# Gustavroot/DeflatedMLMC_Schwinger

Measured on AMD Instinct MI355X. Metric: hutchinson_probe_samples_per_sec_schwinger128, higher is better.
Workload: dtype f64

## Files before the change

deflatedmlmc_schwinger_amd/csrc/sw_engine.hip:

```cpp
#include "../../include/schwinger_hip.h"
#include "sw_kernels.hpp"
#include "sw_pack.hpp"
#include "sw_poly.hpp"

#include <dlfcn.h>

#include <algorithm>
#include <chrono>
#include <cmath>
#include <complex>
#include <cstdarg>
#include <cstdio>
#include <cstdlib>
#include <cstring>
#include <functional>
#include <map>
#include <mutex>
#include <string>
#include <type_traits>
#include <vector>

using swk::cplx;
using swk::cplxf;
using swk::PtrList;
// ... 158 lines not shown
  bool mfma_ops = true;
  bool mfma_3m = true;
  int mfma3_tiles = 0;
  int mfma_tiles = 4;
  int f32_tiles = 0;
  int f32_stages = 4, f32_dense_stages = 8;
  int f32_splitk = 1;
  bool f32_krylov = true;
  bool f32_pairs = true;
  int mfma_small_tiles = 2;
  int sync_hint[SW_MAX_HIER][SW_MAX_LEVELS] = {{0}};
  bool lazy_sync = true;
  int eo_skew = -1;
  bool eo_skew_chunk = false;
  bool gram_cycle = true;
  bool eo_product = true;
  int gj_block = 32;
  int eo_tile = 0;
  int dense_lds = 4;
  int eo_tile_dbg = 0;
  int num_cus = 256;
  bool direct_small = true;
  bool lgmres_aug = true;
  bool stencil_nt = false;
  int stencil_tile = 0;
  int stencil_spw = 0;
  bool cgs2 = false;
  bool verify = true;
  bool inner_cgs2 = false;
  bool pyth_last = true;
// ... 192 lines not shown
    field<&sw_engine::p_even>("p_even"),
    {"ell_order", get_field<&sw_engine::ell_order>, [](sw_engine* h, double v) {
       h->ell_order = v != 0.0;
       for (Hier& H : h->hier) H.even_valid = false;
     }},
    field<&sw_engine::direct_small>("direct_small"),
    field<&sw_engine::eo_direct>("eo_direct"),
    field<&sw_engine::lgmres_aug>("lgmres_aug"),
    field<&sw_engine::cgs2>("cgs2"),
    field<&sw_engine::inner_cgs2>("inner_cgs2"),
    field<&sw_engine::pyth_last>("pyth_last"),
    field<&sw_engine::verify>("verify"),
    field<&sw_engine::lazy_sync>("lazy_sync"),
    field<&sw_engine::eo_solve>("eo_solve"),
    field<&sw_engine::gram_cycle>("gram_cycle"),
    field<&sw_engine::stop_factor>("stop_factor", [](double v) { return v > 0.0 && v <= 1.0; },
                                   "stop_factor must be in (0, 1]"),
    field<&sw_engine::precond_f32>("precond_f32"),
    field<&sw_engine::f32_krylov>("f32_krylov"),
    field<&sw_engine::f32_pairs>("f32_pairs"),
    field<&sw_engine::f32_tiles>("f32_tiles",
                                 [](double v) { const int t = (int)v; return t == 0 || t == 1 || t == 2 || t == 4; },
                                 "f32_tiles must be 0, 1, 2 or 4"),
    field<&sw_engine::f32_stages>("f32_stages"),
    field<&sw_engine::f32_dense_stages>("f32_dense_stages"),
    field<&sw_engine::f32_splitk>("f32_splitk"),
    field<&sw_engine::bench_what>("bench_what", [](double v) { return !(v < 0.0 || v > 3.0); },
                                  "bench_what must be 0..3"),
    field<&sw_engine::bench_mode>("bench_mode", [](double v) { return v == 0.0 || v == 1.0 || v == 2.0; },
                                  "bench_mode must be 0, 1 or 2"),
// ... 901 lines not shown
      const bool even = lv.stencil ? (row < lv.n / 2) : (even_row_tile[row / 16] != 0);
      if (even) ev.push_back(g);
    }
    if (ev.empty()) continue;
    SWCHK(upload(h, &P.order_even, ev.data(), ev.size()));
    P.ngroups_even = (int)ev.size();
  }
  H.even_valid = true;
  return 0;
}

static inline int* sink_slot(sw_engine* h);
static bool f32_capable(const Hier& H, int level);

static int gram_cycle_update(sw_engine* h, const PtrList& pu, const PtrList& pz, int L, int n, int nbp, cplx* X,
                             KrylovWS& ws, swk::FgTail tg) {
  tg.kind = SW_TAIL_GRAM;
  tg.s = ws.sc;
  tg.j = L;
  tg.h1 = ws.gram;
  SWCHK(multigram(h, pu, L + 1, n, nbp, ws.gram, &tg));
  return multiaxpy(h, pz, L, ws.sc.ys, 1.0, X, X, n, nbp, nullptr);
}
static int gram_cycle(sw_engine* h, const KrylovSys& sys, const cplx* R, cplx* X, int L, KrylovWS& ws, int nbp,
                      swk::FgTail tg) {
  const size_t vec = (size_t)sys.n * nbp;
  PtrList pu, pz;
  pu.p[0] = R;
  for (int j = 0; j < L; ++j) {
    cplx* z = ws.Z + vec * j;
    cplx* w = ws.V + vec * j;
    SWCHK(sys.precond(pu.p[j], z));
    SWCHK(sys.apply(0, z, nullptr, w));
    pu.p[j + 1] = w;
    pz.p[j] = z;
  }
  return gram_cycle_update(h, pu, pz, L, sys.n, nbp, X, ws, tg);
}

static int kcycle_gram(sw_engine* h, Hier& H, int level, const cplx* B, cplx* X, int L, KrylovWS& ws, int nbp) {
  swk::FgTail tg{};
  tg.first_cycle = 1;
  tg.notconv = sink_slot(h);
  SWCHK(zero_vec(h, X, H.lv[level].n, nbp));
  return gram_cycle(h, full_system(h, H, level, nbp, true, false), B, X, L, ws, nbp, tg);
}

static int coarse_correction(sw_engine* h, Hier& H, int l, int nbp) {
  Level& lv = H.lv[l];
  Level& lc = H.lv[l + 1];
  const int last = H.nlevels - 1;
  if (lv.kcycle > 0 && l + 1 < last) {
// ... 2199 lines not shown
    return 0;
  }
  if (lv.n <= 0) return sw_fail(h, "level %d undefined", level);
  if (shift >= lv.n) return sw_fail(h, "shift %lld >= n", (long long)shift);
  std::vector<int> src(lv.n);
  for (int i = 0; i < lv.n; ++i) {
    const int s = (int)(((int64_t)i - shift + lv.n) % lv.n);
    const int ri = lv.h_rowmap.empty() ? i : lv.h_rowmap[i];
    const int rs = lv.h_rowmap.empty() ? s : lv.h_rowmap[s];
    src[ri] = rs;
  }
  SWCHK(upload(h, &h->perm_src[level], src.data(), src.size()));
  return 0;
}

int sw_set_rhsmap(sw_engine* h, int level, int n, const int64_t* indptr, const int32_t* indices,
                  const double* data) {
  SWCHK(check_hier(h, 0, level, false));
  HIPCHK(hipSetDevice(h->device));
  Level& lv = h->hier[0].lv[level];
  if (lv.n != n) return sw_fail(h, "rhs map size %d != level size %d", n, lv.n);
  SWCHK(free_op(h, h->rhsmap[level]));
  std::vector<int> rows_int;
  if (!lv.h_rowmap.empty()) {
    rows_int.resize(n);
    for (int i = 0; i < n; ++i) rows_int[lv.h_rowmap[i]] = i;
  }
  return build_ell(h, h->rhsmap[level], n, n, indptr, indices, (const std::complex<double>*)data,
                   rows_int, lv.h_rowmap, 1);
}
// ... 464 lines not shown
  if (h->precond_f32 && h->f32_krylov && f32_capable(H, 0)) {
    s.precond32 = [h, &H, nbp](const cplxf* v, cplxf* z) { return vcycle32_even(h, H, v, z, nbp); };
    s.op32 = [h, &lv, nbp](const cplxf* z, cplxf* w) { return schur_apply32(h, lv, z, w, nbp); };
  }
  return s;
}

static int reduced_rhs(sw_engine* h, Level& lv, const cplx* B, KrylovWS& ws, int nbp) {
  PtrList pl;
  pl.p[0] = B;
  const swk::FgTail tbeg = tail_begin(ws, 1);
  SWCHK(multidot(h, pl, 1, B, lv.n, nbp, ws.nrm, nullptr, nullptr, &tbeg));
  return eo_hop<0>(h, lv, B, B, ws.xacc, nbp);
}

static int fgmres_eo(sw_engine* h, Hier& H, const cplx* B, cplx* X, double tol, int maxiter, int m,
                     KrylovWS& ws, int nbp, int* iters_total) {
  Level& lv = H.lv[0];
  SWCHK(ensure_level_ws(h, lv, nbp));
  SWCHK(reduced_rhs(h, lv, B, ws, nbp));
  SWCHK(fgmres_loop(h, H, 0, reduced_system(h, H, nbp), ws.xacc, X, tol, maxiter, m, true, ws, nbp,
                    iters_total));
  return eo_hop<1>(h, lv, B, X, X, nbp);
}

static int fgmres_eo_gram(sw_engine* h, Hier& H, const cplx* B, cplx* X, double tol, int maxiter, int m,
                          KrylovWS& ws, int nbp, int* iters_total) {
  Level& lv = H.lv[0];
  const int hid_idx = (int)(&H - &h->hier[0]);
  const int hint = h->lazy_sync ? h->sync_hint[hid_idx][0] : 0;
  const KrylovSys sys = reduced_system(h, H, nbp);
  const double tol_stop = tol * h->stop_factor;
  SWCHK(ensure_level_ws(h, lv, nbp));
  SWCHK(reset_slots(h));
  SWCHK(reduced_rhs(h, lv, B, ws, nbp));
  const cplx* bp = ws.xacc;
  SWCHK(zero_vec(h, X, sys.n, nbp));
  std::vector<std::complex<double>> hrr(nbp), hrr0(nbp);
  int done = 0;
  bool converged = false;
  const cplx* Rcur = bp;
  int L = std::min(m, maxiter);
  while (done < maxiter && !converged) {
    L = std::max(1, std::min(L, std::min(m, maxiter - done)));
    int* slot = nullptr;
    SWCHK(take_slot(h, &slot));
    swk::FgTail tg{};
    tg.tol = tol;
    tg.tol_stop = tol_stop;
    tg.iter_base = done;
    tg.notconv = slot;
    SWCHK(gram_cycle(h, sys, Rcur, X, L, ws, nbp, tg));
    done += L;
    SWCHK(sys.apply(1, X, bp, ws.rres));
    Rcur = ws.rres;
    const bool observe = tol_stop > 0.0 && (hint <= 0 || done + m >= hint || done >= maxiter);
    int Lnext = m;
    if (observe) {
      int left = 0;
      SWCHK(read_slot(h, slot, &left));
      if (left == 0) {
        converged = true;
      } else {
        HIPCHK(hipMemcpy(hrr.data(), ws.sc.relres, sizeof(cplx) * nbp, hipMemcpyDeviceToHost));
        HIPCHK(hipMemcpy(hrr0.data(), ws.sc.g, sizeof(cplx) * nbp, hipMemcpyDeviceToHost));
        double need = 1.0;
        for (int c = 0; c < nbp; ++c) {
// ... 9 lines not shown
      PtrList pr;
      pr.p[0] = ws.rres;
      int* vslot = nullptr;
      SWCHK(take_slot(h, &vslot));
      const swk::FgTail tv = tail_verify(ws, tol, tol_stop, vslot);
      SWCHK(multidot(h, pr, 1, ws.rres, sys.n, nbp, ws.nrm, nullptr, nullptr, &tv));
      int left = 0;
      SWCHK(read_slot(h, vslot, &left));
      if (left != 0) {
        converged = false;
        Lnext = 1;
      }
    }
    L = Lnext;
  }
  SWCHK(eo_hop<1>(h, lv, B, X, X, nbp));
  if (iters_total) *iters_total = done;
  h->sync_hint[hid_idx][0] = converged ? done : 0;
  return 0;
}

static bool level_is_direct(sw_engine* h, Hier& H, int level) {
  return h->direct_small && level < H.nlevels - 1 && !H.lv[level].stencil && H.lv[level].dinv.set &&
         h->use_mfma;
}

static int solve_dev(sw_engine* h, int hid, int level0, const cplx* B, cplx* X, double tol,
                     int maxiter, int nbp, int* total) {
  Hier& H = h->hier[hid];
  Level& lv = H.lv[level0];
  if (level0 == H.nlevels - 1 && H.nlevels > 1) {
// ... 1726 lines not shown
  }
  return 0;
}

static int batch_tail(sw_engine* h, const Batch& b, int total, int G, std::initializer_list<ResultBuf*> results,
                      std::vector<int32_t> sum = {}) {
  SWCHK(stream_sync(h));
  for (ResultBuf* r : results) r->done(b.nb);
  sum.resize(b.nb, 0);
  SWCHK(fold_iters(h, b, total, G, sum));
  h->last_iters_f = sum;
  h->last_iters_c.assign(b.nb, 0);
  return 0;
}

static int body_hutchinson(sw_engine* h, const Batch& b) {
  int total = 0;
  SWCHK(pack_probes(h, b));
  SWCHK(fine_solve(h, b, true, &total));
  SWCHK(dot_into(h, h->pb_x0, h->pb_z, h->hier[0].lv[0].n, b.nbp, h->pb_est));
  return batch_tail(h, b, total, 1, {});
}

static int body_shifts(sw_engine* h, const Batch& b) {
  int total = 0;
  SWCHK(pack_probes(h, b));
  SWCHK(fine_solve(h, b, false, &total));
  SWCHK(shift_dots(h, h->hier[0].lv[0], h->pb_probes, b.nb, h->pb_z, b.nbp));
  HIPCHK(hipMemcpyAsync(h->pb_est, h->r_shifts.p, sizeof(cplx) * b.nbp, hipMemcpyDeviceToDevice, h->stream));
  return batch_tail(h, b, total, 1, {&h->r_shifts});
}

// ... 193 lines not shown
  if (m == std::end(kModes)) return sw_fail(h, "unknown mode %d", mode);
  if (m->level0 && level != 0) return sw_fail(h, "%s mode runs at level 0", m->level0);
  if (m->ready) SWCHK(m->ready(h, level));
  Batch b{mode, level, 0, level, h->pb_nb, h->pb_nbp, tol, maxiter};
  SWCHK(solve_hier(h, level, &b.hid));
  if (m->diff == 2 && level != 0) return sw_fail(h, "level skipping is defined for level 0 only");
  if (m->diff) SWCHK(diff_levels(h, level, m->diff == 2, &b.hid, &b.lcoarse));
  HIPCHK(hipSetDevice(h->device));
  SWCHK(ensure_probe_ws(h, b.nbp));
  SWCHK(ensure_small(h, b.nbp));
  if (h->pb_slot >= 0 && h->pb_slot < (int)h->slots.size() && h->slots[h->pb_slot].pending) {
    HIPCHK(hipStreamWaitEvent(h->stream, h->slots[h->pb_slot].ready, 0));
    h->slots[h->pb_slot].pending = false;
  }
  return m->body(h, b);
}


namespace {
struct RcclUid {
  char internal[128];
};
struct Rccl {
  void* lib = nullptr;
  int (*get_uid)(RcclUid*) = nullptr;
  int (*init_rank)(void**, int, RcclUid, int) = nullptr;
  int (*all_reduce)(const void*, void*, size_t, int, int, void*, hipStream_t) = nullptr;
  int (*destroy)(void*) = nullptr;
  bool tried = false, ok = false;
};
// ... 215 lines not shown
```

deflatedmlmc_schwinger_amd/csrc/sw_kernels.hpp:

```cpp
#pragma once
#include <hip/hip_runtime.h>
#include <stdint.h>

namespace swk {

typedef double2 cplx;

#define SW_WAVE 64
#define SW_BLOCK 256
#define SW_WAVES_PER_BLOCK 4
#define SW_SHIFT_SMALL_L 256
#define SW_SHIFT_MID_L 768
#define SW_SHIFT_MAX_L 1024

__device__ __forceinline__ cplx cmake(double a, double b) { cplx r; r.x = a; r.y = b; return r; }
__device__ __forceinline__ cplx cadd(cplx a, cplx b) { return cmake(a.x + b.x, a.y + b.y); }
__device__ __forceinline__ cplx csub(cplx a, cplx b) { return cmake(a.x - b.x, a.y - b.y); }
__device__ __forceinline__ cplx cmul(cplx a, cplx b) {
  return cmake(fma(a.x, b.x, -a.y * b.y), fma(a.x, b.y, a.y * b.x));
}
__device__ __forceinline__ cplx cmulc(cplx a, cplx b) {
  return cmake(fma(a.x, b.x, a.y * b.y), fma(a.x, b.y, -a.y * b.x));
}
__device__ __forceinline__ void cfma(cplx& acc, cplx a, cplx b) {
// ... 2114 lines not shown
  cplx s = cadd(cadd(s0, s1), cadd(s2, s3));
  if (wave > 0) red[wave - 1][lane] = s;
  __syncthreads();
  if (wave == 0) {
    s = cadd(s, red[0][lane]);
    s = cadd(s, red[1][lane]);
    s = cadd(s, red[2][lane]);
    out[(size_t)k * nbp + col] = s;
    if (svec) {
      const double q = svec[(size_t)k * nbp + col].x;
      coef[(size_t)k * nbp + col] = cmake(q * q * s.x, q * q * s.y);
    }
  }
}

template <int KT, bool NORM, class CV = cplx, class CW = cplx>
__global__ __launch_bounds__(SW_BLOCK) void k_multiaxpy(PtrListT<CV> V, int K,
                                                        const cplx* __restrict__ coef, double sign,
                                                        const CW* __restrict__ Win,
                                                        CW* __restrict__ Wout, int n, int nbp,
                                                        int rows_per_block,
                                                        cplx* __restrict__ partial,
                                                        cplxf* __restrict__ W32, RedArgs ra, FgTail tail) {
  __shared__ double redn[3][64];
  __shared__ cplx redt[NORM ? 256 : 1];
  const int wave = threadIdx.x >> 6, lane = threadIdx.x & 63;
  const size_t col = (size_t)blockIdx.y * 64 + lane;
  const int r0 = blockIdx.x * rows_per_block;
  const int r1 = min(n, r0 + rows_per_block);
  cplx c[KT];
#pragma unroll
  for (int k = 0; k < KT; ++k) {
    c[k] = cmake(0.0, 0.0);
    if (k < K) {
      const cplx t = coef[(size_t)k * nbp + col];
      c[k] = cmake(sign * t.x, sign * t.y);
    }
  }
  double nrm = 0.0;
  constexpr int UNR = (sizeof(CV) == sizeof(cplxf) && sizeof(CW) == sizeof(cplxf)) ? 4 : 2;
#pragma unroll UNR
  for (int r = r0 + wave; r < r1; r += SW_WAVES_PER_BLOCK) {
    const size_t off = (size_t)r * nbp + col;
    cplx w = widen(Win[off]);
#pragma unroll
    for (int k = 0; k < KT; ++k)
      if (k < K) cfma(w, c[k], widen(V.p[k][off]));
    Wout[off] = narrow<CW>(w);
    if (W32) W32[off] = cmake((float)w.x, (float)w.y);
    if (NORM) nrm = fma(w.x, w.x, fma(w.y, w.y, nrm));
  }
  if (NORM) {
    if (wave > 0) redn[wave - 1][lane] = nrm;
    __syncthreads();
    if (wave == 0) {
      nrm += redn[0][lane];
      nrm += redn[1][lane];
      nrm += redn[2][lane];
      st_partial(&partial[(size_t)blockIdx.x * nbp + col], cmake(nrm, 0.0), ra.tick1 != nullptr);
// ... 99 lines not shown
                                                         const cplx* __restrict__ X,
                                                         cplx* __restrict__ out, int n, int nbp) {
  const int wave = threadIdx.x >> 6, lane = threadIdx.x & 63;
  const size_t col = (size_t)blockIdx.y * 64 + lane;
  const int r = __builtin_amdgcn_readfirstlane(blockIdx.x * SW_WAVES_PER_BLOCK + wave);
  if (r >= n) return;
  const int s = srcrow ? srcrow[r] : r;
  cplx x = X[(size_t)s * nbp + col];
  const cplx* u = U + (size_t)s * ldu;
#pragma unroll 4
  for (int k = 0; k < kd; ++k) {
    const cplx ck = c[(size_t)k * nbp + col];
    cfma(x, cmake(-u[k].x, -u[k].y), ck);
  }
  out[(size_t)r * nbp + col] = x;
}

template <int KT>
__global__ __launch_bounds__(SW_BLOCK) void k_defl_gemm_dots(const cplx* __restrict__ U, int ldu,
                                                             const cplx* __restrict__ X, int n, int nbp,
                                                             int rows_per_block,
                                                             cplx* __restrict__ partial) {
  const int lane = threadIdx.x & 63, wave = threadIdx.x >> 6;
  const int k = lane >> 4, c = lane & 15;
  const int t0 = wave * KT;
  const int nt = min(KT, ldu / 16 - t0);
  if (nt <= 0) return;
  const int r0 = blockIdx.x * rows_per_block;
  const int r1 = min(n, r0 + rows_per_block);
  const size_t j = (size_t)blockIdx.y * 16 + c;
// ... 1744 lines not shown
```

deflatedmlmc_schwinger_amd/engine.py:

```python
import ctypes as C
import os
import sys

import numpy as np
import scipy.sparse as sp

_HERE = os.path.dirname(os.path.abspath(__file__))
LIB_PATH = os.path.join(_HERE, "libschwinger_hip.so")

MODE_HUTCHINSON = 0
MODE_MLMC = 1
MODE_MLMC_SKIP = 2
MODE_LEVEL = 3
MODE_HUTCHINSON_SHIFTS = 4
MODE_HUTCHINSON_LOOPS = 5
MODE_TWO_POINT = 6
MODE_MLMC_LOOPS = 7
MODE_MLMC_LOOPS_SKIP = 8
MODE_MLMC_DEFL_LOOPS = 9
MODE_MLMC_DEFL_LOOPS_SKIP = 10
MODE_TWO_POINT_LMA = 11
MODE_HUTCHINSON_LINK_LOOPS = 12
MODE_THREE_POINT = 13
MODE_TWO_POINT_SMEARED = 14
# ... 124 lines not shown
    sig("sw_setup_eo_operators", i32, vp, i32, i32, i32)
    sig("sw_apply_eo_operator", i32, vp, i32, i32, i32, i32, vp, vp)
    sig("sw_get_level_bsr", i32, vp, i32, i32, P(i32), vp, vp)
    sig("sw_setup_testvectors", i32, vp, i32, i32, i32, C.c_uint64, i32, dbl, i32, i32, vp)
    sig("sw_setup_transfer", i32, vp, i32, i32, i32, i32, vp, i32, i32, vp, vp, vp)
    sig("sw_setup_galerkin", i32, vp, i32, i32, i32, vp)
    sig("sw_get_level_dense", i32, vp, i32, i32, vp)
    sig("sw_setup_invert_coarsest", i32, vp, i32)
    sig("sw_setup_direct_level", i32, vp, i32, i32)
    sig("sw_setup_level_inverse", i32, vp, i32, i32)
    sig("sw_setup_arnoldi", i32, vp, i32, i32, i32, i32, C.c_uint64, vp)
    sig("sw_hier_end", i32, vp, i32)
    sig("sw_set_deflation", i32, vp, i32, vp)
    sig("sw_set_level_deflation", i32, vp, i32, i32, vp)
    sig("sw_set_perm", i32, vp, i32, i64)
    sig("sw_set_rhsmap", i32, vp, i32, i32, vp, vp, vp)
    sig("sw_set_solver", i32, vp, i32, i32)
    sig("sw_set_option", i32, vp, C.c_char_p, dbl)
    sig("sw_get_option", i32, vp, C.c_char_p, P(dbl))
    sig("sw_pool_trim", i32)
    sig("sw_get_coarsest_inv", i32, vp, i32, vp)
    sig("sw_eig_begin", i32, vp, i32, i32, C.c_uint64)
    sig("sw_eig_begin_wide", i32, vp, i32, i32, C.c_uint64, i32)
    sig("sw_eig_load", i32, vp, i32, i32, vp)
    sig("sw_eig_solve", i32, vp, i32, i32, i32, dbl, i32, P(i32))
    sig("sw_eig_apply_diff", i32, vp, i32, i32, i32, i32, dbl, i32, P(i32))
    sig("sw_eig_gram", i32, vp, i32, i32, vp)
    sig("sw_eig_rotate", i32, vp, i32, vp, i32, i32)
    sig("sw_eig_fetch", i32, vp, i32, i32, vp)
    sig("sw_eig_end", i32, vp)
# ... 10 lines not shown
        P(i32), vp)
    sig("sw_krylov_multiaxpy", i32, vp, i32, i32, i32, i32, i32, i32, vp, vp, dbl, vp, vp, vp, vp)
    sig("sw_krylov_scalars", i32, vp, i32, i32, i32, i32, i32, dbl, dbl, i32, vp, vp, vp, vp, vp, P(i32))
    sig("sw_solve", i32, vp, i32, i32, i32, vp, vp, dbl, i32, vp, vp)
    sig("sw_hutch_batch", i32, vp, i32, i32, i32, vp, dbl, i32, vp, vp)
    sig("sw_probes_upload", i32, vp, i32, i32, vp)
    sig("sw_probes_upload_slot", i32, vp, i32, i32, i32, vp)
    sig("sw_probes_select", i32, vp, i32)
    sig("sw_kernel_stats", i32, vp, i32, P(dbl), P(i64))
    sig("sw_kernel_work", i32, vp, i32, P(dbl))
    sig("sw_comm_unique_id", i32, vp)
    sig("sw_comm_init", i32, vp, i32, i32, vp)
    sig("sw_allreduce_stats", i32, vp, vp)
    sig("sw_comm_destroy", i32, vp)
    sig("sw_hutch_run", i32, vp, i32, i32, dbl, i32)
    sig("sw_sync", i32, vp)
    sig("sw_hutch_fetch", i32, vp, vp, vp)
    sig("sw_bench_dirac", i32, vp, i32, i32, i32, i32, P(dbl))
    sig("sw_set_profiling", i32, vp, i32)
    sig("sw_timers", i32, vp, P(dbl))
    sig("sw_timers_reset", i32, vp)
    sig("sw_launch_count", i32, vp, P(i64))
    sig("sw_mt_create", vp, C.c_uint32)
    sig("sw_mt_destroy", None, vp)
    sig("sw_mt_skip", None, vp, C.c_uint64)
    sig("sw_mt_raw", None, vp, C.c_uint64, vp)
    sig("sw_mt_rademacher", None, vp, C.c_uint64, vp)
    sig("sw_mt_z4", None, vp, C.c_uint64, vp)
    sig("sw_mt_from_state", vp, vp, i32)
    sig("sw_mt_get_state", None, vp, vp, P(i32))
# ... 39 lines not shown
    sig("sw_set_distillation_momenta", i32, vp, i32, vp)
    sig("sw_apply_laph_elementals", i32, vp, vp)
    sig("sw_distilled_two_point", i32, vp, i32, vp, dbl, i32, vp, vp, vp, vp)
    sig("sw_apply_laph_contract", i32, vp, i32, vp, vp, vp, vp)
    sig("sw_generalized_perambulators", i32, vp, i32, i32, i32, vp, i32, vp, dbl, i32, vp, vp, vp)
    sig("sw_apply_laph_generalized", i32, vp, i32, vp, i32, vp, i32, vp, i32, vp, vp)
    _lib = lib
    return lib


EXPORTED_SYMBOLS = (
    "sw_create", "sw_destroy", "sw_last_error", "sw_device_count", "sw_version", "sw_hier_begin",
    "sw_set_lattice", "sw_set_csr", "sw_set_transfer", "sw_set_coarsest_inv", "sw_set_cycle",
    "sw_set_smoother", "sw_set_gmres_smoother", "sw_set_eo_smoother", "sw_set_eo_operator", "sw_setup_eo_operators", "sw_apply_eo_operator",
    "sw_get_level_bsr", "sw_setup_testvectors", "sw_setup_transfer",
    "sw_setup_galerkin", "sw_get_level_dense", "sw_setup_invert_coarsest", "sw_setup_direct_level", "sw_setup_level_inverse", "sw_setup_arnoldi", "sw_hier_end", "sw_set_deflation", "sw_set_level_deflation", "sw_set_perm", "sw_set_rhsmap", "sw_set_solver", "sw_set_option", "sw_get_option",
    "sw_pool_trim", "sw_get_coarsest_inv", "sw_eig_begin", "sw_eig_begin_wide", "sw_eig_load", "sw_eig_solve", "sw_eig_apply_diff", "sw_eig_gram", "sw_eig_rotate", "sw_eig_fetch", "sw_eig_end",
    "sw_apply_dirac", "sw_restrict", "sw_prolong", "sw_coarsest", "sw_apply_deflation", "sw_vcycle", "sw_apply_op32", "sw_apply_op64", "sw_solve",
    "sw_krylov_multidot", "sw_krylov_gram_cycle", "sw_krylov_multiaxpy", "sw_krylov_scalars",
    "sw_hutch_batch", "sw_probes_upload", "sw_probes_upload_slot", "sw_probes_select",
    "sw_kernel_stats", "sw_kernel_work", "sw_hutch_run", "sw_sync", "sw_hutch_fetch",
    "sw_comm_unique_id", "sw_comm_init", "sw_allreduce_stats", "sw_comm_destroy",
    "sw_bench_dirac", "sw_set_profiling", "sw_timers", "sw_timers_reset", "sw_launch_count",
    "sw_mt_create", "sw_mt_destroy", "sw_mt_skip", "sw_mt_raw", "sw_mt_rademacher",
    "sw_mt_z4", "sw_mt_from_state", "sw_mt_get_state", "sw_mt_window", "sw_mt_jump",
    "sw_mt_jump_poly", "sw_mt_window_jump",
    "sw_probes_stream_set", "sw_probes_generate", "sw_probes_fetch",
    "sw_set_shifts", "sw_hutch_fetch_shifts", "sw_apply_shift_dots",
    "sw_set_loop_momenta", "sw_hutch_fetch_loops", "sw_apply_slice_dots",
    "sw_set_two_point", "sw_hutch_fetch_two_point", "sw_apply_slice_sources", "sw_apply_pair_dots",
    "sw_apply_slice_cdots", "sw_coarsest_loops", "sw_hutch_fetch_mlmc_loops", "sw_level_deflation_loops",
    "sw_meson_fields", "sw_low_mode_two_point", "sw_set_low_mode_inverse", "sw_apply_low_mode", "sw_hutch_fetch_two_point_lma",
    "sw_hutch_fetch_link_loops", "sw_apply_slice_link_dots",
    "sw_set_three_point", "sw_hutch_fetch_three_point", "sw_apply_seq_sources", "sw_apply_seq_dots",
    "sw_set_smearing", "sw_apply_smearing", "sw_hutch_fetch_two_point_smeared",
    "sw_set_distillation", "sw_perambulators", "sw_apply_laph_sources", "sw_apply_laph_project",
# ... 238 lines not shown
        Y = np.empty_like(X2)
        self._chk(self._lib.sw_apply_low_mode(self._h, X2.shape[0], _ptr(X2), _ptr(Y)), "sw_apply_low_mode")
        return Y[0] if single else Y

    def set_level_deflation(self, level, V):
        if V is None:
            self._chk(self._lib.sw_set_level_deflation(self._h, level, 0, None),
                      "sw_set_level_deflation")
            return
        V = _c128(np.asarray(V))
        self._chk(self._lib.sw_set_level_deflation(self._h, level, V.shape[1], _ptr(V)),
                  "sw_set_level_deflation")

    def set_perm(self, level, shift):
        self._chk(self._lib.sw_set_perm(self._h, level, int(shift)), "sw_set_perm")

    def set_shifts(self, shifts):
        s = np.ascontiguousarray([] if shifts is None else shifts, dtype=np.int64).ravel()
        self._chk(self._lib.sw_set_shifts(self._h, s.size, _ptr(s) if s.size else None), "sw_set_shifts")
        self._nshifts = int(s.size)

    def set_loop_momenta(self, momenta):
        p = np.ascontiguousarray([] if momenta is None else momenta, dtype=np.int32).ravel()
        self._chk(self._lib.sw_set_loop_momenta(self._h, p.size, _ptr(p) if p.size else None),
                  "sw_set_loop_momenta")
        self._nmom = int(p.size)

    def set_rhsmap(self, level, Cmat):
        (n, m), indptr, indices, data = _csr_parts(Cmat)
        self._chk(self._lib.sw_set_rhsmap(self._h, level, n, _ptr(indptr), _ptr(indices),
# ... 608 lines not shown
        ms = C.c_double(0.0)
        cnt = C.c_int64(0)
        self._chk(self._lib.sw_kernel_stats(self._h, which, C.byref(ms), C.byref(cnt)),
                  "sw_kernel_stats")
        return ms.value, int(cnt.value)

    def kernel_work(self, which):
        w = C.c_double(0.0)
        self._chk(self._lib.sw_kernel_work(self._h, which, C.byref(w)), "sw_kernel_work")
        return w.value

    def hutch_run(self, mode, level, tol, maxiter=1000):
        self._chk(self._lib.sw_hutch_run(self._h, mode, level, float(tol), int(maxiter)),
                  "sw_hutch_run")

    def sync(self):
        self._chk(self._lib.sw_sync(self._h), "sw_sync")

    def hutch_fetch(self):
        nb = self._nb_uploaded
        ests = np.zeros(nb, dtype=np.complex128)
        iters = np.zeros(2 * nb, dtype=np.int32)
        self._chk(self._lib.sw_hutch_fetch(self._h, _ptr(ests), _ptr(iters)), "sw_hutch_fetch")
        return ests, iters[:nb].copy(), iters[nb:].copy()

    @staticmethod
    def comm_unique_id():
        buf = C.create_string_buffer(128)
        if load_library().sw_comm_unique_id(buf) != 0:
            raise EngineError("sw_comm_unique_id failed (RCCL not loadable)")
# ... 107 lines not shown
```

include/schwinger_hip.h:

```cpp
#ifndef SCHWINGER_HIP_H
#define SCHWINGER_HIP_H

#include <stdint.h>

#ifdef __cplusplus
extern "C" {
#endif

#define SW_MAX_HIER 2
#define SW_MAX_LEVELS 8
#define SW_MAX_KRYLOV 32
#define SW_MAX_DEFL 256
#define SW_MAX_SHIFTS 128
#define SW_MAX_MOMENTA 8
#define SW_MAX_SINK_LEVELS 4
#define SW_MAX_SMEARING_STEPS 1024
#define SW_MAX_LAPH 128

typedef struct sw_engine sw_engine;

int sw_create(sw_engine** out, int device_id);
int sw_destroy(sw_engine* h);
const char* sw_last_error(sw_engine* h);
int sw_device_count(void);
// ... 32 lines not shown
int sw_eig_begin_wide(sw_engine* h, int hid, int level, uint64_t seed, int width);
int sw_eig_load(sw_engine* h, int dst, int ncols, const double* X);
int sw_eig_solve(sw_engine* h, int src, int dst, int mode, double tol, int maxiter, int32_t* iters_max);
int sw_eig_apply_diff(sw_engine* h, int src, int dst, int skip, int g3, double tol, int maxiter,
                      int32_t* iters_max);
int sw_eig_gram(sw_engine* h, int a, int b, double* out);
int sw_eig_rotate(sw_engine* h, int src, const double* Y, int dst, int sub);
int sw_eig_fetch(sw_engine* h, int src, int k, double* out);
int sw_eig_end(sw_engine* h);
int sw_hier_end(sw_engine* h, int hid);

int sw_set_deflation(sw_engine* h, int k, const double* U);
int sw_set_low_mode_inverse(sw_engine* h, int k, const double* G);
int sw_set_level_deflation(sw_engine* h, int level, int k, const double* V);
int sw_set_perm(sw_engine* h, int level, int64_t shift);
int sw_set_rhsmap(sw_engine* h, int level, int n, const int64_t* indptr, const int32_t* indices,
                  const double* data);
int sw_set_shifts(sw_engine* h, int nshifts, const int64_t* shifts);
int sw_set_loop_momenta(sw_engine* h, int nmom, const int32_t* p);
int sw_set_two_point(sw_engine* h, int t0, int nmom, const int32_t* p);
int sw_set_smearing(sw_engine* h, double kappa, int source_steps, int nsink, const int32_t* sink_steps);
int sw_set_distillation(sw_engine* h, int nev, const double* V);
int sw_set_three_point(sw_engine* h, int t0, int tf, int sink_gamma, int pf, int nmom, const int32_t* q);
int sw_set_solver(sw_engine* h, int restart, int solver_hid);

int sw_set_option(sw_engine* h, const char* name, double value);
int sw_get_option(sw_engine* h, const char* name, double* value);

int sw_apply_dirac(sw_engine* h, int hid, int level, int nb, const double* X, double* Y);
int sw_restrict(sw_engine* h, int hid, int level, int nb, const double* X, double* Y);
// ... 81 lines not shown
#define SW_MODE_TWO_POINT_LMA 11
#define SW_MODE_HUTCHINSON_LINK_LOOPS 12
#define SW_MODE_THREE_POINT 13
#define SW_MODE_TWO_POINT_SMEARED 14
int sw_hutch_batch(sw_engine* h, int mode, int level, int nb, const int8_t* probes, double tol,
                   int maxiter, double* ests, int32_t* iters);
int sw_probes_upload(sw_engine* h, int level, int nb, const int8_t* probes);
int sw_probes_upload_slot(sw_engine* h, int slot, int level, int nb, const int8_t* probes);
int sw_probes_select(sw_engine* h, int slot);
#define SW_PROBES_Z2 1
#define SW_PROBES_Z4 2
int sw_probes_stream_set(sw_engine* h, const uint32_t* window);
int sw_probes_generate(sw_engine* h, int slot, int level, int nb, int kind, uint64_t pos);
int sw_probes_fetch(sw_engine* h, int slot, int8_t* out);
int sw_hutch_run(sw_engine* h, int mode, int level, double tol, int maxiter);
int sw_sync(sw_engine* h);
int sw_hutch_fetch(sw_engine* h, double* ests, int32_t* iters);
int sw_hutch_fetch_shifts(sw_engine* h, double* ests);
int sw_hutch_fetch_loops(sw_engine* h, double* out);
int sw_hutch_fetch_mlmc_loops(sw_engine* h, double* out);
int sw_hutch_fetch_link_loops(sw_engine* h, double* out);
int sw_hutch_fetch_two_point(sw_engine* h, double* out);
int sw_hutch_fetch_two_point_lma(sw_engine* h, double* out);
int sw_hutch_fetch_three_point(sw_engine* h, double* out);
int sw_hutch_fetch_two_point_smeared(sw_engine* h, double* out);

int sw_comm_unique_id(char id[128]);
int sw_comm_init(sw_engine* h, int nranks, int rank, const char id[128]);
int sw_allreduce_stats(sw_engine* h, double stats[4]);
int sw_comm_destroy(sw_engine* h);
// ... 47 lines not shown
```

Measured before the change: 35800.

## Fuse Hutchinson probe deflation, reduced RHS and estimate into int8-code kernels

For plain Hutchinson batches on level 0 with deflation, the probe packing, deflation, even-odd reduced RHS and the final odd reconstruction plus dot product are replaced by kernels that read the int8 probe codes directly. Deflation coefficients come from a new int8 dot kernel, and the estimate is accumulated inside the odd-site hop kernel. The first gram cycle also skips zeroing X and reading it back in the multiaxpy. The aim is to cut full-vector memory passes and kernel launches per batch. In exchange it adds recomputation of deflated probe values per stencil neighbour and stricter eligibility conditions.

```diff
diff --git a/deflatedmlmc_schwinger_amd/csrc/sw_engine.hip b/deflatedmlmc_schwinger_amd/csrc/sw_engine.hip
--- a/deflatedmlmc_schwinger_amd/csrc/sw_engine.hip
+++ b/deflatedmlmc_schwinger_amd/csrc/sw_engine.hip
@@ -196,6 +196,7 @@
   int eo_skew = -1;
   bool eo_skew_chunk = false;
   bool gram_cycle = true;
+  bool batch_ends = true;
   bool eo_product = true;
   int gj_block = 32;
   int eo_tile = 0;
@@ -418,6 +419,7 @@
     field<&sw_engine::lazy_sync>("lazy_sync"),
     field<&sw_engine::eo_solve>("eo_solve"),
     field<&sw_engine::gram_cycle>("gram_cycle"),
+    field<&sw_engine::batch_ends>("batch_ends"),
     field<&sw_engine::stop_factor>("stop_factor", [](double v) { return v > 0.0 && v <= 1.0; },
                                    "stop_factor must be in (0, 1]"),
     field<&sw_engine::precond_f32>("precond_f32"),
@@ -1349,16 +1351,24 @@
 static bool f32_capable(const Hier& H, int level);
 
 static int gram_cycle_update(sw_engine* h, const PtrList& pu, const PtrList& pz, int L, int n, int nbp, cplx* X,
-                             KrylovWS& ws, swk::FgTail tg) {
+                             KrylovWS& ws, swk::FgTail tg, bool x_zero = false) {
   tg.kind = SW_TAIL_GRAM;
   tg.s = ws.sc;
   tg.j = L;
   tg.h1 = ws.gram;
   SWCHK(multigram(h, pu, L + 1, n, nbp, ws.gram, &tg));
-  return multiaxpy(h, pz, L, ws.sc.ys, 1.0, X, X, n, nbp, nullptr);
+  if (!x_zero) return multiaxpy(h, pz, L, ws.sc.ys, 1.0, X, X, n, nbp, nullptr);
+  int P, rpb;
+  row_blocking(n, nbp, false, &P, &rpb);
+  const swk::RedArgs ra{};
+  return pick_ge<2, 4>(L, [&](auto KT) {
+    return launch(h, T_AXPY, swk::k_multiaxpy<KT, false, cplx, cplx, true>, dim3(P, nbp / 64), dim3(SW_BLOCK), pz, L,
+                  (const cplx*)ws.sc.ys, 1.0, (const cplx*)nullptr, X, n, nbp, rpb, h->partial, (cplxf*)nullptr, ra,
+                  kNoTail);
+  });
 }
 static int gram_cycle(sw_engine* h, const KrylovSys& sys, const cplx* R, cplx* X, int L, KrylovWS& ws, int nbp,
-                      swk::FgTail tg) {
+                      swk::FgTail tg, bool x_zero = false) {
   const size_t vec = (size_t)sys.n * nbp;
   PtrList pu, pz;
   pu.p[0] = R;
@@ -1370,7 +1380,7 @@
     pu.p[j + 1] = w;
     pz.p[j] = z;
   }
-  return gram_cycle_update(h, pu, pz, L, sys.n, nbp, X, ws, tg);
+  return gram_cycle_update(h, pu, pz, L, sys.n, nbp, X, ws, tg, x_zero);
 }
 
 static int kcycle_gram(sw_engine* h, Hier& H, int level, const cplx* B, cplx* X, int L, KrylovWS& ws, int nbp) {
@@ -3600,6 +3610,23 @@
   return 0;
 }
 
+int sw_set_perm_table(sw_engine* h, int level, int n, const int32_t* src) {
+  SWCHK(check_hier(h, 0, level, false));
+  HIPCHK(hipSetDevice(h->device));
+  Level& lv = h->hier[0].lv[level];
+  if (!src) return sw_fail(h, "null gather table");
+  if (lv.n <= 0 || lv.n != n) return sw_fail(h, "gather table of %d rows, level %d has %d", n, level, lv.n);
+  std::vector<int> tab(n);
+  for (int i = 0; i < n; ++i) {
+    if (src[i] < 0 || src[i] >= n) return sw_fail(h, "gather table entry %d = %d outside [0,%d)", i, src[i], n);
+    const int ri = lv.h_rowmap.empty() ? i : lv.h_rowmap[i];
+    tab[ri] = lv.h_rowmap.empty() ? src[i] : lv.h_rowmap[src[i]];
+  }
+  SWCHK(stream_sync(h));
+  SWCHK(upload(h, &h->perm_src[level], tab.data(), tab.size()));
+  return 0;
+}
+
 int sw_set_rhsmap(sw_engine* h, int level, int n, const int64_t* indptr, const int32_t* indices,
                   const double* data) {
   SWCHK(check_hier(h, 0, level, false));
@@ -4094,6 +4121,48 @@
   return eo_hop<0>(h, lv, B, B, ws.xacc, nbp);
 }
 
+struct BatchEnds {
+  swk::DeflRows d;
+  cplx* est;
+};
+static void ends_blocking(int Vh, int* P, int* spw) {
+  auto blocks = [&](int s) { return ((Vh + s - 1) / s + SW_WAVES_PER_BLOCK - 1) / SW_WAVES_PER_BLOCK; };
+  int s = 4;
+  while (blocks(s) > SW_RED_GROUP * SW_RED_MAXGROUPS) s *= 2;
+  *spw = s;
+  *P = blocks(s);
+}
+static const auto pick_ends = [](int kd, auto&& f) {
+  if (kd <= 8) return f(IntC<8>{});
+  if (kd <= 16) return f(IntC<16>{});
+  return f(IntC<0>{});
+};
+static int ends_rhs(sw_engine* h, Level& lv, const BatchEnds& be, KrylovWS& ws, int nbp) {
+  const swk::StencilArgs a = stencil_args<cplx>(h, lv, nbp, true);
+  int P, spw;
+  ends_blocking(a.Vh, &P, &spw);
+  const int ngroups = (P + SW_RED_GROUP - 1) / SW_RED_GROUP;
+  SWCHK(ensure_partial(h, (size_t)(P + ngroups) * nbp * sizeof(cplx)));
+  const swk::RedArgs ra = red_args(h, true, P, 1, nbp, ws.nrm, nullptr, nullptr);
+  const swk::FgTail tbeg = tail_begin(ws, 1);
+  return pick_ends(be.d.kd, [&](auto KT) {
+    return launch(h, T_SCHUR, swk::k_rhs_even_i8<KT>, dim3(P, nbp / 64), dim3(SW_BLOCK), be.d, ws.xacc, a, 1.0,
+                  1.0 / a.diag, spw, h->partial, ra, tbeg);
+  });
+}
+static int ends_estimate(sw_engine* h, Level& lv, const BatchEnds& be, const cplx* X, int nbp) {
+  const swk::StencilArgs a = stencil_args<cplx>(h, lv, nbp, true);
+  int P, spw;
+  ends_blocking(a.Vh, &P, &spw);
+  const int ngroups = (P + SW_RED_GROUP - 1) / SW_RED_GROUP;
+  SWCHK(ensure_partial(h, (size_t)(P + ngroups) * nbp * sizeof(cplx)));
+  const swk::RedArgs ra = red_args(h, true, P, 1, nbp, be.est, nullptr, nullptr);
+  return pick_ends(be.d.kd, [&](auto KT) {
+    return launch(h, T_DOTS, swk::k_est_odd_i8<KT>, dim3(P, nbp / 64), dim3(SW_BLOCK), be.d, X, a,
+                  1.0 / a.diag, 1.0 / a.diag, spw, h->partial, ra, kNoTail);
+  });
+}
+
 static int fgmres_eo(sw_engine* h, Hier& H, const cplx* B, cplx* X, double tol, int maxiter, int m,
                      KrylovWS& ws, int nbp, int* iters_total) {
   Level& lv = H.lv[0];
@@ -4105,7 +4174,7 @@
 }
 
 static int fgmres_eo_gram(sw_engine* h, Hier& H, const cplx* B, cplx* X, double tol, int maxiter, int m,
-                          KrylovWS& ws, int nbp, int* iters_total) {
+                          KrylovWS& ws, int nbp, int* iters_total, const BatchEnds* ends = nullptr) {
   Level& lv = H.lv[0];
   const int hid_idx = (int)(&H - &h->hier[0]);
   const int hint = h->lazy_sync ? h->sync_hint[hid_idx][0] : 0;
@@ -4113,9 +4182,10 @@
   const double tol_stop = tol * h->stop_factor;
   SWCHK(ensure_level_ws(h, lv, nbp));
   SWCHK(reset_slots(h));
-  SWCHK(reduced_rhs(h, lv, B, ws, nbp));
+  if (ends) SWCHK(ends_rhs(h, lv, *ends, ws, nbp));
+  else SWCHK(reduced_rhs(h, lv, B, ws, nbp));
   const cplx* bp = ws.xacc;
-  SWCHK(zero_vec(h, X, sys.n, nbp));
+  if (!ends) SWCHK(zero_vec(h, X, sys.n, nbp));
   std::vector<std::complex<double>> hrr(nbp), hrr0(nbp);
   int done = 0;
   bool converged = false;
@@ -4130,7 +4200,7 @@
     tg.tol_stop = tol_stop;
     tg.iter_base = done;
     tg.notconv = slot;
-    SWCHK(gram_cycle(h, sys, Rcur, X, L, ws, nbp, tg));
+    SWCHK(gram_cycle(h, sys, Rcur, X, L, ws, nbp, tg, ends && done == 0));
     done += L;
     SWCHK(sys.apply(1, X, bp, ws.rres));
     Rcur = ws.rres;
@@ -4170,7 +4240,8 @@
     }
     L = Lnext;
   }
-  SWCHK(eo_hop<1>(h, lv, B, X, X, nbp));
+  if (ends) SWCHK(ends_estimate(h, lv, *ends, X, nbp));
+  else SWCHK(eo_hop<1>(h, lv, B, X, X, nbp));
   if (iters_total) *iters_total = done;
   h->sync_hint[hid_idx][0] = converged ? done : 0;
   return 0;
@@ -5927,8 +5998,66 @@
   return 0;
 }
 
+static bool hutch_ends_eligible(sw_engine* h, const Batch& b) {
+  if (!h->batch_ends || b.mode != SW_MODE_HUTCHINSON || b.level != 0) return false;
+  if (h->kd < 1 || h->kd > 64 || h->defl_gemm || !h->U) return false;
+  Hier& H = h->hier[b.hid];
+  if (H.nlevels < 2 || level_is_direct(h, H, 0) || h->precond_f32 || !h->gram_cycle) return false;
+  if (!eo_solve_eligible(h, H, 0)) return false;
+  Level& lv = H.lv[0];
+  const int m = std::min(h->restart, std::max(1, b.maxiter));
+  int P = 0, rpb = 0, Pe = 0, spw = 0;
+  row_blocking(lv.n / 2, b.nbp, true, &P, &rpb);
+  ends_blocking(lv.L * lv.L / 2, &Pe, &spw);
+  return m <= SW_GRAM_MAXL && fused_ok(h, P, b.nbp) && fused_ok(h, Pe, b.nbp) && lv.n == 2 * lv.L * lv.L &&
+         h->hier[0].lv[0].n == lv.n;
+}
+
+static int ends_coeffs(sw_engine* h, int n, int nbp, cplx* cbuf) {
+  const int kd = h->kd, ld = defl_ld(kd);
+  int P, rpb;
+  row_blocking(n, nbp, true, &P, &rpb);
+  for (int k0 = 0; k0 < kd; k0 += 32) {
+    const int kc = std::min(32, kd - k0);
+    SWCHK(ensure_partial(h, (size_t)P * kc * nbp * sizeof(cplx)));
+    SWCHK(pick_ge<8, 16, 32>(kc, [&](auto KC) {
+      return launch(h, T_DEFL, swk::k_defl_dots_i8<KC>, dim3(P, nbp / 64), dim3(SW_BLOCK), (const cplx*)(h->U + k0),
+                    ld, kc, (const int8_t*)h->pb_codes, n, nbp, rpb, h->partial);
+    }));
+    SWCHK(launch(h, T_DEFL, swk::k_reduce_partials, dim3(kc, nbp / 64), dim3(SW_BLOCK), h->partial, P, kc, nbp,
+                 cbuf + (size_t)k0 * nbp, (const cplx*)nullptr, (cplx*)nullptr));
+  }
+  return 0;
+}
+
+static int ends_begin(sw_engine* h, const Batch& b, BatchEnds* be) {
+  Level& lv = h->hier[0].lv[0];
+  SWCHK(launch(h, T_OTHER, swk::k_probe_codes, dim3((lv.n + 63) / 64, b.nbp / 64), dim3(SW_BLOCK), h->pb_probes,
+               b.nb, lv.n, (const int*)lv.rowmap, h->pb_codes, b.nbp));
+  cplx* cbuf = h->small + 8 * b.nbp;
+  SWCHK(ends_coeffs(h, lv.n, b.nbp, cbuf));
+  be->d.codes = h->pb_codes;
+  be->d.U = h->U;
+  be->d.c = cbuf;
+  be->d.srcrow = h->perm_src[0];
+  be->d.ldu = defl_ld(h->kd);
+  be->d.kd = h->kd;
+  be->est = h->pb_est;
+  return 0;
+}
+
 static int body_hutchinson(sw_engine* h, const Batch& b) {
   int total = 0;
+  if (hutch_ends_eligible(h, b)) {
+    Hier& H = h->hier[b.hid];
+    Level& lv = H.lv[0];
+    BatchEnds be;
+    SWCHK(ends_begin(h, b, &be));
+    const int m = std::min(h->restart, std::max(1, b.maxiter));
+    SWCHK(ensure_krylov(h, lv.sws, m, lv.n, b.nbp, true));
+    SWCHK(fgmres_eo_gram(h, H, nullptr, h->pb_z, b.tol, b.maxiter, m, lv.sws, b.nbp, &total, &be));
+    return batch_tail(h, b, total, 1, {});
+  }
   SWCHK(pack_probes(h, b));
   SWCHK(fine_solve(h, b, true, &total));
   SWCHK(dot_into(h, h->pb_x0, h->pb_z, h->hier[0].lv[0].n, b.nbp, h->pb_est));
@@ -6152,6 +6281,47 @@
     h->slots[h->pb_slot].pending = false;
   }
   return m->body(h, b);
+}
+
+int sw_hutch_rhs_debug(sw_engine* h, int which, double tol, int maxiter, double* c, double* bpe, double* normb) {
+  SWCHK(check_hier(h, 0, 0, true));
+  if (which != 0 && which != 1) return sw_fail(h, "which must be 0 (stored) or 1 (from the codes)");
+  if (h->pb_level != 0 || h->pb_nb <= 0) return sw_fail(h, "no probes uploaded for level 0");
+  if (h->kd <= 0 || !h->U) return sw_fail(h, "no deflation vectors registered (sw_set_deflation)");
+  if (maxiter < 1 || !c || !bpe || !normb) return sw_fail(h, "bad arguments");
+  Batch b{SW_MODE_HUTCHINSON, 0, 0, 0, h->pb_nb, h->pb_nbp, tol, maxiter};
+  SWCHK(solve_hier(h, 0, &b.hid));
+  HIPCHK(hipSetDevice(h->device));
+  SWCHK(ensure_probe_ws(h, b.nbp));
+  SWCHK(ensure_small(h, b.nbp));
+  if (h->pb_slot >= 0 && h->pb_slot < (int)h->slots.size() && h->slots[h->pb_slot].pending) {
+    HIPCHK(hipStreamWaitEvent(h->stream, h->slots[h->pb_slot].ready, 0));
+    h->slots[h->pb_slot].pending = false;
+  }
+  Hier& H = h->hier[b.hid];
+  Level& lv = H.lv[0];
+  if (!eo_solve_eligible(h, H, 0)) return sw_fail(h, "the even-odd reduced solve is not eligible here");
+  const int m = std::min(h->restart, std::max(1, maxiter)), nbp = b.nbp, n = lv.n;
+  SWCHK(ensure_krylov(h, lv.sws, m, n, nbp, true));
+  SWCHK(ensure_level_ws(h, lv, nbp));
+  KrylovWS& ws = lv.sws;
+  if (which == 1) {
+    if (!hutch_ends_eligible(h, b)) return sw_fail(h, "this batch would not take its ends from the codes");
+    BatchEnds be;
+    SWCHK(ends_begin(h, b, &be));
+    SWCHK(ends_rhs(h, lv, be, ws, nbp));
+  } else {
+    SWCHK(pack_probes(h, b));
+    SWCHK(deflate(h, h->U, h->kd, (const int*)h->perm_src[0], h->pb_x0, h->pb_rhs, n, nbp));
+    SWCHK(reduced_rhs(h, lv, h->pb_rhs, ws, nbp));
+  }
+  SWCHK(stream_sync(h));
+  HIPCHK(hipMemcpy(c, h->small + 8 * nbp, sizeof(cplx) * nbp * h->kd, hipMemcpyDeviceToHost));
+  HIPCHK(hipMemcpy(bpe, ws.xacc, sizeof(cplx) * nbp * (n / 2), hipMemcpyDeviceToHost));
+  std::vector<std::complex<double>> nn(nbp);
+  HIPCHK(hipMemcpy(nn.data(), ws.sc.normb, sizeof(cplx) * nbp, hipMemcpyDeviceToHost));
+  for (int j = 0; j < nbp; ++j) normb[j] = nn[j].real();
+  return 0;
 }
 
 
diff --git a/deflatedmlmc_schwinger_amd/csrc/sw_kernels.hpp b/deflatedmlmc_schwinger_amd/csrc/sw_kernels.hpp
--- a/deflatedmlmc_schwinger_amd/csrc/sw_kernels.hpp
+++ b/deflatedmlmc_schwinger_amd/csrc/sw_kernels.hpp
@@ -2152,7 +2152,7 @@
   }
 }
 
-template <int KT, bool NORM, class CV = cplx, class CW = cplx>
+template <int KT, bool NORM, class CV = cplx, class CW = cplx, bool ZERO = false>
 __global__ __launch_bounds__(SW_BLOCK) void k_multiaxpy(PtrListT<CV> V, int K,
                                                         const cplx* __restrict__ coef, double sign,
                                                         const CW* __restrict__ Win,
@@ -2180,7 +2180,7 @@
 #pragma unroll UNR
   for (int r = r0 + wave; r < r1; r += SW_WAVES_PER_BLOCK) {
     const size_t off = (size_t)r * nbp + col;
-    cplx w = widen(Win[off]);
+    cplx w = ZERO ? cmake(0.0, 0.0) : widen(Win[off]);
 #pragma unroll
     for (int k = 0; k < KT; ++k)
       if (k < K) cfma(w, c[k], widen(V.p[k][off]));
@@ -2310,6 +2310,205 @@
     cfma(x, cmake(-u[k].x, -u[k].y), ck);
   }
   out[(size_t)r * nbp + col] = x;
+}
+
+__device__ __forceinline__ cplx code_cplx(int v) {
+  return (v == 2 || v == -2) ? cmake(0.0, (double)(v / 2)) : cmake((double)v, 0.0);
+}
+
+template <int KT>
+__global__ __launch_bounds__(SW_BLOCK) void k_defl_dots_i8(const cplx* __restrict__ U, int ldu, int kd,
+                                                           const int8_t* __restrict__ codes, int n, int nbp,
+                                                           int rows_per_block, cplx* __restrict__ partial) {
+  __shared__ cplx red[3][8][64];
+  const int wave = threadIdx.x >> 6, lane = threadIdx.x & 63;
+  const size_t col = (size_t)blockIdx.y * 64 + lane;
+  const int r0 = blockIdx.x * rows_per_block;
+  const int r1 = min(n, r0 + rows_per_block);
+  cplx acc[KT];
+#pragma unroll
+  for (int k = 0; k < KT; ++k) acc[k] = cmake(0.0, 0.0);
+  int r = __builtin_amdgcn_readfirstlane(r0 + wave);
+  for (; r + 3 * SW_WAVES_PER_BLOCK < r1; r += 4 * SW_WAVES_PER_BLOCK) {
+    int cd[4];
+#pragma unroll
+    for (int i = 0; i < 4; ++i) cd[i] = codes[(size_t)(r + i * SW_WAVES_PER_BLOCK) * nbp + col];
+#pragma unroll
+    for (int i = 0; i < 4; ++i) {
+      const cplx x = code_cplx(cd[i]);
+      const cplx* u = U + (size_t)(r + i * SW_WAVES_PER_BLOCK) * ldu;
+#pragma unroll
+      for (int k = 0; k < KT; ++k)
+        if (k < kd) cfmac(acc[k], u[k], x);
+    }
+  }
+  for (; r < r1; r += SW_WAVES_PER_BLOCK) {
+    const cplx x = code_cplx(codes[(size_t)r * nbp + col]);
+    const cplx* u = U + (size_t)r * ldu;
+#pragma unroll
+    for (int k = 0; k < KT; ++k)
+      if (k < kd) cfmac(acc[k], u[k], x);
+  }
+  for (int kb = 0; kb < KT; kb += 8) {
+    if (kb >= kd) break;
+    if (wave > 0) {
+#pragma unroll
+      for (int k = 0; k < 8; ++k)
+        if (kb + k < KT) red[wave - 1][k][lane] = acc[kb + k];
+    }
+    __syncthreads();
+    if (wave == 0) {
+#pragma unroll
+      for (int k = 0; k < 8; ++k) {
+        if (kb + k < KT && kb + k < kd) {
+          cplx s = acc[kb + k];
+          s = cadd(s, red[0][k][lane]);
+          s = cadd(s, red[1][k][lane]);
+          s = cadd(s, red[2][k][lane]);
+          partial[((size_t)blockIdx.x * kd + kb + k) * nbp + col] = s;
+        }
+      }
+    }
+    __syncthreads();
+  }
+}
+
+struct DeflRows {
+  const int8_t* codes;
+  const cplx* U;
+  const cplx* c;
+  const int* srcrow;
+  int ldu, kd;
+};
+template <int KT>
+struct DeflCoef {
+  cplx c[KT > 0 ? KT : 1];
+  __device__ __forceinline__ void load(const DeflRows& d, int nbp, size_t col) {
+#pragma unroll
+    for (int k = 0; k < KT; ++k) c[k] = (k < d.kd) ? d.c[(size_t)k * nbp + col] : cmake(0.0, 0.0);
+  }
+};
+template <int KT>
+__device__ __forceinline__ cplx defl_row(const DeflRows& d, const DeflCoef<KT>& cc, int r, int nbp, size_t col) {
+  const int s = d.srcrow ? d.srcrow[r] : r;
+  cplx x = code_cplx(d.codes[(size_t)s * nbp + col]);
+  const cplx* u = d.U + (size_t)s * d.ldu;
+  if (KT > 0) {
+#pragma unroll
+    for (int k = 0; k < KT; ++k)
+      if (k < d.kd) cfma(x, cmake(-u[k].x, -u[k].y), cc.c[k]);
+  } else {
+#pragma unroll 4
+    for (int k = 0; k < d.kd; ++k) {
+      const cplx ck = d.c[(size_t)k * nbp + col];
+      cfma(x, cmake(-u[k].x, -u[k].y), ck);
+    }
+  }
+  return x;
+}
+template <int KT>
+__device__ __forceinline__ Site2 defl_site(const DeflRows& d, const DeflCoef<KT>& cc, int x, int y, int L, int Vh,
+                                           int nbp, size_t col) {
+  const int r = (int)eo_row(x, y, L, Vh);
+  Site2 v;
+  v.s0 = defl_row<KT>(d, cc, r, nbp, col);
+  v.s1 = defl_row<KT>(d, cc, r + 1, nbp, col);
+  return v;
+}
+
+template <int KT>
+__global__ __launch_bounds__(SW_BLOCK) void k_rhs_even_i8(DeflRows d, cplx* __restrict__ out, StencilArgs a,
+                                                          double alpha, double beta, int spw,
+                                                          cplx* __restrict__ partial, RedArgs ra, FgTail tail) {
+  __shared__ double redn[3][64];
+  __shared__ cplx redt[256];
+  const int wave = threadIdx.x >> 6, lane = threadIdx.x & 63;
+  const int L = a.L, Vh = a.Vh, nbp = a.nbp;
+  const size_t col = (size_t)blockIdx.y * 64 + lane;
+  const int w = __builtin_amdgcn_readfirstlane(xcd_remap(blockIdx.x, gridDim.x) * SW_WAVES_PER_BLOCK + wave);
+  DeflCoef<KT> cc;
+  cc.load(d, nbp, col);
+  double nrm = 0.0;
+  for (int i = 0; i < spw; ++i) {
+    const int sh = w * spw + i;
+    if (sh >= Vh) break;
+    int x, y;
+    eo_site(sh, 0, L, a.tile_w, 0, L, x, y);
+    const int xp = wrap_p(x, L), xm = wrap_m(x, L), yp = wrap_p(y, L), ym = wrap_m(y, L);
+    Site2 acc;
+    acc.s0 = cmake(0.0, 0.0);
+    acc.s1 = acc.s0;
+    const Site2 bxp = defl_site<KT>(d, cc, xp, y, L, Vh, nbp, col);
+    hop_acc<0>(acc, a.U1[y * L + x], bxp);
+    hop_acc<1>(acc, a.U1[y * L + xm], defl_site<KT>(d, cc, xm, y, L, Vh, nbp, col));
+    hop_acc<2>(acc, a.U2[y * L + x], defl_site<KT>(d, cc, x, yp, L, Vh, nbp, col));
+    hop_acc<3>(acc, a.U2[ym * L + x], defl_site<KT>(d, cc, x, ym, L, Vh, nbp, col));
+    const Site2 own = defl_site<KT>(d, cc, x, y, L, Vh, nbp, col);
+    const size_t r = eo_row(x, y, L, Vh);
+    out[r * nbp + col] = clin(alpha, own.s0, beta, acc.s0);
+    out[(r + 1) * nbp + col] = clin(alpha, own.s1, beta, acc.s1);
+    nrm = fma(own.s0.x, own.s0.x, fma(own.s0.y, own.s0.y, nrm));
+    nrm = fma(own.s1.x, own.s1.x, fma(own.s1.y, own.s1.y, nrm));
+    nrm = fma(bxp.s0.x, bxp.s0.x, fma(bxp.s0.y, bxp.s0.y, nrm));
+    nrm = fma(bxp.s1.x, bxp.s1.x, fma(bxp.s1.y, bxp.s1.y, nrm));
+  }
+  if (wave > 0) redn[wave - 1][lane] = nrm;
+  __syncthreads();
+  if (wave == 0) {
+    nrm += redn[0][lane];
+    nrm += redn[1][lane];
+    nrm += redn[2][lane];
+    st_partial(&partial[(size_t)blockIdx.x * nbp + col], cmake(nrm, 0.0), true);
+  }
+  reduce_and_tail<1>(partial, 1, nbp, ra, tail, redt);
+}
+
+template <int KT>
+__global__ __launch_bounds__(SW_BLOCK) void k_est_odd_i8(DeflRows d, const cplx* __restrict__ X, StencilArgs a,
+                                                         double alpha, double beta, int spw,
+                                                         cplx* __restrict__ partial, RedArgs ra, FgTail tail) {
+  __shared__ cplx redn[3][64];
+  __shared__ cplx redt[256];
+  const int wave = threadIdx.x >> 6, lane = threadIdx.x & 63;
+  const int L = a.L, Vh = a.Vh, nbp = a.nbp;
+  const size_t col = (size_t)blockIdx.y * 64 + lane;
+  const int w = __builtin_amdgcn_readfirstlane(xcd_remap(blockIdx.x, gridDim.x) * SW_WAVES_PER_BLOCK + wave);
+  DeflCoef<KT> cc;
+  cc.load(d, nbp, col);
+  const cplx* Xc = X + col;
+  cplx est = cmake(0.0, 0.0);
+  for (int i = 0; i < spw; ++i) {
+    const int sh = w * spw + i;
+    if (sh >= Vh) break;
+    int x, y;
+    eo_site(sh, 1, L, a.tile_w, 0, L, x, y);
+    const int xp = wrap_p(x, L), xm = wrap_m(x, L), yp = wrap_p(y, L), ym = wrap_m(y, L);
+    Site2 acc;
+    acc.s0 = cmake(0.0, 0.0);
+    acc.s1 = acc.s0;
+    const Site2 exm = ld_site(Xc, xm, y, L, Vh, nbp);
+    hop_acc<0>(acc, a.U1[y * L + x], ld_site(Xc, xp, y, L, Vh, nbp));
+    hop_acc<1>(acc, a.U1[y * L + xm], exm);
+    hop_acc<2>(acc, a.U2[y * L + x], ld_site(Xc, x, yp, L, Vh, nbp));
+    hop_acc<3>(acc, a.U2[ym * L + x], ld_site(Xc, x, ym, L, Vh, nbp));
+    const Site2 bo = defl_site<KT>(d, cc, x, y, L, Vh, nbp, col);
+    const cplx z0 = clin(alpha, bo.s0, beta, acc.s0);
+    const cplx z1 = clin(alpha, bo.s1, beta, acc.s1);
+    const size_t r = eo_row(x, y, L, Vh), re = eo_row(xm, y, L, Vh);
+    cfmac(est, code_cplx(d.codes[r * nbp + col]), z0);
+    cfmac(est, code_cplx(d.codes[(r + 1) * nbp + col]), z1);
+    cfmac(est, code_cplx(d.codes[re * nbp + col]), exm.s0);
+    cfmac(est, code_cplx(d.codes[(re + 1) * nbp + col]), exm.s1);
+  }
+  if (wave > 0) redn[wave - 1][lane] = est;
+  __syncthreads();
+  if (wave == 0) {
+    est = cadd(est, redn[0][lane]);
+    est = cadd(est, redn[1][lane]);
+    est = cadd(est, redn[2][lane]);
+    st_partial(&partial[(size_t)blockIdx.x * nbp + col], est, true);
+  }
+  reduce_and_tail<1>(partial, 1, nbp, ra, tail, redt);
 }
 
 template <int KT>
diff --git a/deflatedmlmc_schwinger_amd/engine.py b/deflatedmlmc_schwinger_amd/engine.py
--- a/deflatedmlmc_schwinger_amd/engine.py
+++ b/deflatedmlmc_schwinger_amd/engine.py
@@ -162,6 +162,7 @@
     sig("sw_set_deflation", i32, vp, i32, vp)
     sig("sw_set_level_deflation", i32, vp, i32, i32, vp)
     sig("sw_set_perm", i32, vp, i32, i64)
+    sig("sw_set_perm_table", i32, vp, i32, i32, vp)
     sig("sw_set_rhsmap", i32, vp, i32, i32, vp, vp, vp)
     sig("sw_set_solver", i32, vp, i32, i32)
     sig("sw_set_option", i32, vp, C.c_char_p, dbl)
@@ -202,6 +203,7 @@
     sig("sw_allreduce_stats", i32, vp, vp)
     sig("sw_comm_destroy", i32, vp)
     sig("sw_hutch_run", i32, vp, i32, i32, dbl, i32)
+    sig("sw_hutch_rhs_debug", i32, vp, i32, dbl, i32, vp, vp, vp)
     sig("sw_sync", i32, vp)
     sig("sw_hutch_fetch", i32, vp, vp, vp)
     sig("sw_bench_dirac", i32, vp, i32, i32, i32, i32, P(dbl))
@@ -271,12 +273,12 @@
     "sw_set_lattice", "sw_set_csr", "sw_set_transfer", "sw_set_coarsest_inv", "sw_set_cycle",
     "sw_set_smoother", "sw_set_gmres_smoother", "sw_set_eo_smoother", "sw_set_eo_operator", "sw_setup_eo_operators", "sw_apply_eo_operator",
     "sw_get_level_bsr", "sw_setup_testvectors", "sw_setup_transfer",
-    "sw_setup_galerkin", "sw_get_level_dense", "sw_setup_invert_coarsest", "sw_setup_direct_level", "sw_setup_level_inverse", "sw_setup_arnoldi", "sw_hier_end", "sw_set_deflation", "sw_set_level_deflation", "sw_set_perm", "sw_set_rhsmap", "sw_set_solver", "sw_set_option", "sw_get_option",
+    "sw_setup_galerkin", "sw_get_level_dense", "sw_setup_invert_coarsest", "sw_setup_direct_level", "sw_setup_level_inverse", "sw_setup_arnoldi", "sw_hier_end", "sw_set_deflation", "sw_set_level_deflation", "sw_set_perm", "sw_set_perm_table", "sw_set_rhsmap", "sw_set_solver", "sw_set_option", "sw_get_option",
     "sw_pool_trim", "sw_get_coarsest_inv", "sw_eig_begin", "sw_eig_begin_wide", "sw_eig_load", "sw_eig_solve", "sw_eig_apply_diff", "sw_eig_gram", "sw_eig_rotate", "sw_eig_fetch", "sw_eig_end",
     "sw_apply_dirac", "sw_restrict", "sw_prolong", "sw_coarsest", "sw_apply_deflation", "sw_vcycle", "sw_apply_op32", "sw_apply_op64", "sw_solve",
     "sw_krylov_multidot", "sw_krylov_gram_cycle", "sw_krylov_multiaxpy", "sw_krylov_scalars",
     "sw_hutch_batch", "sw_probes_upload", "sw_probes_upload_slot", "sw_probes_select",
-    "sw_kernel_stats", "sw_kernel_work", "sw_hutch_run", "sw_sync", "sw_hutch_fetch",
+    "sw_kernel_stats", "sw_kernel_work", "sw_hutch_run", "sw_hutch_rhs_debug", "sw_sync", "sw_hutch_fetch",
     "sw_comm_unique_id", "sw_comm_init", "sw_allreduce_stats", "sw_comm_destroy",
     "sw_bench_dirac", "sw_set_profiling", "sw_timers", "sw_timers_reset", "sw_launch_count",
     "sw_mt_create", "sw_mt_destroy", "sw_mt_skip", "sw_mt_raw", "sw_mt_rademacher",
@@ -545,6 +547,10 @@
 
     def set_perm(self, level, shift):
         self._chk(self._lib.sw_set_perm(self._h, level, int(shift)), "sw_set_perm")
+
+    def set_perm_table(self, level, src):
+        s = np.ascontiguousarray(src, dtype=np.int32).ravel()
+        self._chk(self._lib.sw_set_perm_table(self._h, int(level), s.size, _ptr(s)), "sw_set_perm_table")
 
     def set_shifts(self, shifts):
         s = np.ascontiguousarray([] if shifts is None else shifts, dtype=np.int64).ravel()
@@ -1183,6 +1189,16 @@
         self._chk(self._lib.sw_hutch_run(self._h, mode, level, float(tol), int(maxiter)),
                   "sw_hutch_run")
 
+    def hutch_rhs_debug(self, which, kd, tol, maxiter=1000):
+        n = self.level_sizes[0][0]
+        nbp = (self._nb_uploaded + 63) // 64 * 64
+        c = np.zeros((kd, nbp), dtype=np.complex128)
+        bpe = np.zeros((n // 2, nbp), dtype=np.complex128)
+        normb = np.zeros(nbp, dtype=np.float64)
+        self._chk(self._lib.sw_hutch_rhs_debug(self._h, int(which), float(tol), int(maxiter), _ptr(c), _ptr(bpe),
+                                               _ptr(normb)), "sw_hutch_rhs_debug")
+        return c, bpe, normb
+
     def sync(self):
         self._chk(self._lib.sw_sync(self._h), "sw_sync")
 
diff --git a/include/schwinger_hip.h b/include/schwinger_hip.h
--- a/include/schwinger_hip.h
+++ b/include/schwinger_hip.h
@@ -70,6 +70,7 @@
 int sw_set_low_mode_inverse(sw_engine* h, int k, const double* G);
 int sw_set_level_deflation(sw_engine* h, int level, int k, const double* V);
 int sw_set_perm(sw_engine* h, int level, int64_t shift);
+int sw_set_perm_table(sw_engine* h, int level, int n, const int32_t* src);
 int sw_set_rhsmap(sw_engine* h, int level, int n, const int64_t* indptr, const int32_t* indices,
                   const double* data);
 int sw_set_shifts(sw_engine* h, int nshifts, const int64_t* shifts);
@@ -181,6 +182,7 @@
 int sw_probes_generate(sw_engine* h, int slot, int level, int nb, int kind, uint64_t pos);
 int sw_probes_fetch(sw_engine* h, int slot, int8_t* out);
 int sw_hutch_run(sw_engine* h, int mode, int level, double tol, int maxiter);
+int sw_hutch_rhs_debug(sw_engine* h, int which, double tol, int maxiter, double* c, double* bpe, double* normb);
 int sw_sync(sw_engine* h);
 int sw_hutch_fetch(sw_engine* h, double* ests, int32_t* iters);
 int sw_hutch_fetch_shifts(sw_engine* h, double* ests);
```

Result: no change. 36220, median of 6 (+1.2%).
